# qucontrol/krotov

Hardware: AMD Instinct MI355X
Metric: state*timestep propagations/s (Krotov iterations/s in iterations_per_sec), 256-objective N=64 ensemble (higher is better)
Workload: dtype f64

## Files before the change

krotov_amd/csrc/kh_instances.inc:

```
#if KH_TU == KH_TU_MAIN
extern template __global__ void kh_coop_sweep_store<16, 16, false>(KhSweepArgs, KhCoopArgs, KhExchange, double const*, HIP_vector_type<double, 2u> const*, HIP_vector_type<double, 2u>*, HIP_vector_type<double, 2u>*, int);
extern template __global__ void kh_coop_sweep_store<16, 2, false>(KhSweepArgs, KhCoopArgs, KhExchange, double const*, HIP_vector_type<double, 2u> const*, HIP_vector_type<double, 2u>*, HIP_vector_type<double, 2u>*, int);
extern template __global__ void kh_coop_sweep_store<16, 2, true>(KhSweepArgs, KhCoopArgs, KhExchange, double const*, HIP_vector_type<double, 2u> const*, HIP_vector_type<double, 2u>*, HIP_vector_type<double, 2u>*, int);
extern template __global__ void kh_coop_sweep_store<16, 4, false>(KhSweepArgs, KhCoopArgs, KhExchange, double const*, HIP_vector_type<double, 2u> const*, HIP_vector_type<double, 2u>*, HIP_vector_type<double, 2u>*, int);
extern template __global__ void kh_coop_sweep_store<16, 4, true>(KhSweepArgs, KhCoopArgs, KhExchange, double const*, HIP_vector_type<double, 2u> const*, HIP_vector_type<double, 2u>*, HIP_vector_type<double, 2u>*, int);
extern template __global__ void kh_coop_sweep_store<8, 16, false>(KhSweepArgs, KhCoopArgs, KhExchange, double const*, HIP_vector_type<double, 2u> const*, HIP_vector_type<double, 2u>*, HIP_vector_type<double, 2u>*, int);
extern template __global__ void kh_coop_sweep_store<8, 16, true>(KhSweepArgs, KhCoopArgs, KhExchange, double const*, HIP_vector_type<double, 2u> const*, HIP_vector_type<double, 2u>*, HIP_vector_type<double, 2u>*, int);
extern template __global__ void kh_coop_sweep_store<8, 2, false>(KhSweepArgs, KhCoopArgs, KhExchange, double const*, HIP_vector_type<double, 2u> const*, HIP_vector_type<double, 2u>*, HIP_vector_type<double, 2u>*, int);
extern template __global__ void kh_coop_sweep_store<8, 2, true>(KhSweepArgs, KhCoopArgs, KhExchange, double const*, HIP_vector_type<double, 2u> const*, HIP_vector_type<double, 2u>*, HIP_vector_type<double, 2u>*, int);
extern template __global__ void kh_coop_sweep_store<8, 4, false>(KhSweepArgs, KhCoopArgs, KhExchange, double const*, HIP_vector_type<double, 2u> const*, HIP_vector_type<double, 2u>*, HIP_vector_type<double, 2u>*, int);
extern template __global__ void kh_coop_sweep_store<8, 4, true>(KhSweepArgs, KhCoopArgs, KhExchange, double const*, HIP_vector_type<double, 2u> const*, HIP_vector_type<double, 2u>*, HIP_vector_type<double, 2u>*, int);
extern template __global__ void kh_coop_forward_update<16, 16, false, false, false, true>(KhSweepArgs, KhCoopArgs, KhUpdateArgs, KhExchange);
extern template __global__ void kh_coop_forward_update<16, 2, false, false, false, true>(KhSweepArgs, KhCoopArgs, KhUpdateArgs, KhExchange);
extern template __global__ void kh_coop_forward_update<16, 2, false, true, true, false>(KhSweepArgs, KhCoopArgs, KhUpdateArgs, KhExchange);
extern template __global__ void kh_coop_forward_update<16, 2, true, false, false, true>(KhSweepArgs, KhCoopArgs, KhUpdateArgs, KhExchange);
extern template __global__ void kh_coop_forward_update<16, 4, false, false, false, true>(KhSweepArgs, KhCoopArgs, KhUpdateArgs, KhExchange);
extern template __global__ void kh_coop_forward_update<16, 4, false, true, true, false>(KhSweepArgs, KhCoopArgs, KhUpdateArgs, KhExchange);
extern template __global__ void kh_coop_forward_update<16, 4, true, false, false, true>(KhSweepArgs, KhCoopArgs, KhUpdateArgs, KhExchange);
extern template __global__ void kh_coop_forward_update<8, 16, false, false, false, true>(KhSweepArgs, KhCoopArgs, KhUpdateArgs, KhExchange);
extern template __global__ void kh_coop_forward_update<8, 16, false, true, true, false>(KhSweepArgs, KhCoopArgs, KhUpdateArgs, KhExchange);
extern template __global__ void kh_coop_forward_update<8, 16, true, false, false, true>(KhSweepArgs, KhCoopArgs, KhUpdateArgs, KhExchange);
extern template __global__ void kh_coop_forward_update<8, 2, false, false, false, true>(KhSweepArgs, KhCoopArgs, KhUpdateArgs, KhExchange);
extern template __global__ void kh_coop_forward_update<8, 2, false, true, true, false>(KhSweepArgs, KhCoopArgs, KhUpdateArgs, KhExchange);
extern template __global__ void kh_coop_forward_update<8, 2, true, false, false, true>(KhSweepArgs, KhCoopArgs, KhUpdateArgs, KhExchange);
// ... 75 lines not shown
extern template __global__ void kh_lind_forward_update<2>(KhSweepArgs, KhLindArgs, KhUpdateArgs, KhExchange);
extern template __global__ void kh_lind_forward_update<4>(KhSweepArgs, KhLindArgs, KhUpdateArgs, KhExchange);
extern template __global__ void kh_lind_sweep_store<1>(KhSweepArgs, KhLindArgs, double const*, HIP_vector_type<double, 2u> const*, HIP_vector_type<double, 2u>*, HIP_vector_type<double, 2u>*, int);
extern template __global__ void kh_lind_sweep_store<2>(KhSweepArgs, KhLindArgs, double const*, HIP_vector_type<double, 2u> const*, HIP_vector_type<double, 2u>*, HIP_vector_type<double, 2u>*, int);
extern template __global__ void kh_lind_sweep_store<4>(KhSweepArgs, KhLindArgs, double const*, HIP_vector_type<double, 2u> const*, HIP_vector_type<double, 2u>*, HIP_vector_type<double, 2u>*, int);
extern template __global__ void kh_mini_forward_update<false>(KhSweepArgs, HIP_vector_type<double, 2u> const* const*, KhUpdateArgs, KhExchange);
extern template __global__ void kh_mini_forward_update<true>(KhSweepArgs, HIP_vector_type<double, 2u> const* const*, KhUpdateArgs, KhExchange);
extern template __global__ void kh_quad_forward_update<false>(KhSweepArgs, HIP_vector_type<double, 2u> const* const*, KhUpdateArgs, KhExchange);
extern template __global__ void kh_quad_forward_update<true>(KhSweepArgs, HIP_vector_type<double, 2u> const* const*, KhUpdateArgs, KhExchange);
extern template __global__ void kh_q2_forward_update<false, false, false>(KhSweepArgs, HIP_vector_type<double, 2u> const* const*, KhUpdateArgs, KhExchange);
extern template __global__ void kh_q2_forward_update<false, false, true>(KhSweepArgs, HIP_vector_type<double, 2u> const* const*, KhUpdateArgs, KhExchange);
extern template __global__ void kh_q2_forward_update<false, true, false>(KhSweepArgs, HIP_vector_type<double, 2u> const* const*, KhUpdateArgs, KhExchange);
extern template __global__ void kh_q2_forward_update<false, true, true>(KhSweepArgs, HIP_vector_type<double, 2u> const* const*, KhUpdateArgs, KhExchange);
extern template __global__ void kh_q2_forward_update<true, false, false>(KhSweepArgs, HIP_vector_type<double, 2u> const* const*, KhUpdateArgs, KhExchange);
extern template __global__ void kh_q2_forward_update<true, false, true>(KhSweepArgs, HIP_vector_type<double, 2u> const* const*, KhUpdateArgs, KhExchange);
extern template __global__ void kh_stream_forward_update<1, false, false>(KhSweepArgs, KhUpdateArgs, KhExchange);
extern template __global__ void kh_stream_forward_update<1, false, true>(KhSweepArgs, KhUpdateArgs, KhExchange);
extern template __global__ void kh_stream_forward_update<1, true, false>(KhSweepArgs, KhUpdateArgs, KhExchange);
extern template __global__ void kh_stream_forward_update<1, true, true>(KhSweepArgs, KhUpdateArgs, KhExchange);
extern template __global__ void kh_stream_forward_update<2, false, false>(KhSweepArgs, KhUpdateArgs, KhExchange);
extern template __global__ void kh_stream_forward_update<2, false, true>(KhSweepArgs, KhUpdateArgs, KhExchange);
extern template __global__ void kh_stream_forward_update<2, true, false>(KhSweepArgs, KhUpdateArgs, KhExchange);
extern template __global__ void kh_stream_forward_update<2, true, true>(KhSweepArgs, KhUpdateArgs, KhExchange);
extern template __global__ void kh_stream_forward_update<3, false, false>(KhSweepArgs, KhUpdateArgs, KhExchange);
extern template __global__ void kh_stream_forward_update<3, false, true>(KhSweepArgs, KhUpdateArgs, KhExchange);
extern template __global__ void kh_stream_forward_update<3, true, false>(KhSweepArgs, KhUpdateArgs, KhExchange);
extern template __global__ void kh_stream_forward_update<3, true, true>(KhSweepArgs, KhUpdateArgs, KhExchange);
extern template __global__ void kh_stream_forward_update<4, false, false>(KhSweepArgs, KhUpdateArgs, KhExchange);
extern template __global__ void kh_stream_forward_update<4, false, true>(KhSweepArgs, KhUpdateArgs, KhExchange);
extern template __global__ void kh_stream_forward_update<4, true, false>(KhSweepArgs, KhUpdateArgs, KhExchange);
// ... 162 lines not shown
template __global__ void kh_lind_sweep_store<1>(KhSweepArgs, KhLindArgs, double const*, HIP_vector_type<double, 2u> const*, HIP_vector_type<double, 2u>*, HIP_vector_type<double, 2u>*, int);
template __global__ void kh_lind_sweep_store<2>(KhSweepArgs, KhLindArgs, double const*, HIP_vector_type<double, 2u> const*, HIP_vector_type<double, 2u>*, HIP_vector_type<double, 2u>*, int);
template __global__ void kh_lind_sweep_store<4>(KhSweepArgs, KhLindArgs, double const*, HIP_vector_type<double, 2u> const*, HIP_vector_type<double, 2u>*, HIP_vector_type<double, 2u>*, int);
#elif KH_TU == KH_TU_MINI
template __global__ void kh_mini_forward_update<false>(KhSweepArgs, HIP_vector_type<double, 2u> const* const*, KhUpdateArgs, KhExchange);
template __global__ void kh_mini_forward_update<true>(KhSweepArgs, HIP_vector_type<double, 2u> const* const*, KhUpdateArgs, KhExchange);
template __global__ void kh_quad_forward_update<false>(KhSweepArgs, HIP_vector_type<double, 2u> const* const*, KhUpdateArgs, KhExchange);
template __global__ void kh_quad_forward_update<true>(KhSweepArgs, HIP_vector_type<double, 2u> const* const*, KhUpdateArgs, KhExchange);
#elif KH_TU == KH_TU_Q2
template __global__ void kh_q2_forward_update<false, false, false>(KhSweepArgs, HIP_vector_type<double, 2u> const* const*, KhUpdateArgs, KhExchange);
template __global__ void kh_q2_forward_update<false, false, true>(KhSweepArgs, HIP_vector_type<double, 2u> const* const*, KhUpdateArgs, KhExchange);
template __global__ void kh_q2_forward_update<false, true, false>(KhSweepArgs, HIP_vector_type<double, 2u> const* const*, KhUpdateArgs, KhExchange);
template __global__ void kh_q2_forward_update<false, true, true>(KhSweepArgs, HIP_vector_type<double, 2u> const* const*, KhUpdateArgs, KhExchange);
template __global__ void kh_q2_forward_update<true, false, false>(KhSweepArgs, HIP_vector_type<double, 2u> const* const*, KhUpdateArgs, KhExchange);
template __global__ void kh_q2_forward_update<true, false, true>(KhSweepArgs, HIP_vector_type<double, 2u> const* const*, KhUpdateArgs, KhExchange);
#elif KH_TU == KH_TU_STREAM
template __global__ void kh_stream_forward_update<1, false, false>(KhSweepArgs, KhUpdateArgs, KhExchange);
template __global__ void kh_stream_forward_update<1, false, true>(KhSweepArgs, KhUpdateArgs, KhExchange);
template __global__ void kh_stream_forward_update<1, true, false>(KhSweepArgs, KhUpdateArgs, KhExchange);
template __global__ void kh_stream_forward_update<1, true, true>(KhSweepArgs, KhUpdateArgs, KhExchange);
template __global__ void kh_stream_forward_update<2, false, false>(KhSweepArgs, KhUpdateArgs, KhExchange);
template __global__ void kh_stream_forward_update<2, false, true>(KhSweepArgs, KhUpdateArgs, KhExchange);
template __global__ void kh_stream_forward_update<2, true, false>(KhSweepArgs, KhUpdateArgs, KhExchange);
template __global__ void kh_stream_forward_update<2, true, true>(KhSweepArgs, KhUpdateArgs, KhExchange);
template __global__ void kh_stream_forward_update<3, false, false>(KhSweepArgs, KhUpdateArgs, KhExchange);
template __global__ void kh_stream_forward_update<3, false, true>(KhSweepArgs, KhUpdateArgs, KhExchange);
template __global__ void kh_stream_forward_update<3, true, false>(KhSweepArgs, KhUpdateArgs, KhExchange);
template __global__ void kh_stream_forward_update<3, true, true>(KhSweepArgs, KhUpdateArgs, KhExchange);
template __global__ void kh_stream_forward_update<4, false, false>(KhSweepArgs, KhUpdateArgs, KhExchange);
template __global__ void kh_stream_forward_update<4, false, true>(KhSweepArgs, KhUpdateArgs, KhExchange);
// ... 58 lines not shown
```

krotov_amd/csrc/kh_tile64q2.h:

```cpp
#pragma once

#include "kh_common.h"
#include "kh_generic.h"
#include "kh_tile64.h"

#define KH_Q2_THREADS 512
#ifdef KH_Q2_DPP_REDUCE
typedef KhLanes<false> KhQ2Lanes;
#else
typedef KhLanes<true> KhQ2Lanes;
#endif
#define KH_Q2_TILE_ELEMS (8 * KH_Q2_THREADS)

struct KhQ2Lds {
    cplx *h0;
    cplx *p0;
    cplx (*buf)[KH_TILE_N];
    cplx *chib;
    cplx *sbuf;
    double *red;
    double *D;
    double2 *inv2;
    double *deg;
};

__host__ __device__ inline size_t kh_q2_lds_bytes() {
    return (size_t)2 * KH_Q2_TILE_ELEMS * sizeof(cplx) + 4 * KH_TILE_N * sizeof(cplx) + (2 * 8 * 2 + 4) * sizeof(double) +
           (KH_MAX_DEGREE / 2 + 1) * sizeof(double2) + (KH_MAX_DEGREE + 2) * sizeof(double);
}

__device__ __forceinline__ KhQ2Lds kh_q2_carve(char *smem) {
    KhQ2Lds s;
    s.h0 = (cplx *)smem;
    s.p0 = s.h0 + KH_Q2_TILE_ELEMS;
    s.buf = (cplx(*)[KH_TILE_N])(s.p0 + KH_Q2_TILE_ELEMS);
    s.chib = (cplx *)(s.buf + 2);
    s.sbuf = s.chib + KH_TILE_N;
    s.red = (double *)(s.sbuf + KH_TILE_N);
    s.D = s.red + 2 * 8 * 2;
    s.inv2 = (double2 *)(s.D + 4);
    s.deg = (double *)(s.inv2 + KH_MAX_DEGREE / 2 + 1);
    return s;
}

__device__ __forceinline__ void kh_q2_load_tile(const cplx *op, int N, int wave, int lane, cplx (&t)[8]) {
    const int row = wave * 8 + KhQ2Lanes::row_in(lane), cg = KhQ2Lanes::cg(lane);
#pragma unroll
    for (int j = 0; j < 8; ++j) {
        const int col = cg + 8 * j;
        t[j] = (op != nullptr && row < N && col < N) ? op[(size_t)row * N + col] : c_make(0.0, 0.0);
    }
}

__device__ __forceinline__ void kh_q2_stage_tile(const cplx *op, int N, int wave, int lane, int tid, cplx *dst) {
    cplx t[8];
    kh_q2_load_tile(op, N, wave, lane, t);
// ... 47 lines not shown

__device__ __forceinline__ void kh_q2_advance(const KhQ2Lds &s, int tid, double eps, double eps_prev, const cplx (&h1)[8],
                                              cplx (&a)[8], cplx (&b)[8]) {
    const double e1 = eps - eps_prev, e2 = e1 * (eps + eps_prev);
#pragma unroll
    for (int j = 0; j < 8; ++j) {
        const cplx q1 = s.h0[j * KH_Q2_THREADS + tid];
        const cplx q2 = s.p0[j * KH_Q2_THREADS + tid];
        a[j].x = fma(e1, h1[j].x, a[j].x);
        a[j].y = fma(e1, h1[j].y, a[j].y);
        b[j].x = fma(e2, q2.x, fma(e1, q1.x, b[j].x));
        b[j].y = fma(e2, q2.y, fma(e1, q1.y, b[j].y));
    }
}

template <class Epilogue>
__device__ __forceinline__ int kh_q2_expm_action(const cplx (&a)[8], const cplx (&b)[8], cplx &state,
                                                 cplx (*buf)[KH_TILE_N], cplx *sbuf, const double2 *inv2, int &cur,
                                                 cplx *store_in, int N, double fre, double fim,
                                                 double dt, int nsub, int m, int wave, int lane,
                                                 Epilogue epilogue) {
    const int cg = KhQ2Lanes::cg(lane), row = wave * 8 + KhQ2Lanes::row_out(lane);
    const bool writer = (lane & 7) == 0;
    const double h = nsub == 1 ? dt : dt / nsub;
    const double f2h2 = (fre * fre - fim * fim) * h * h;
    const int phases = (m + 1) >> 1;
    if (store_in != nullptr && wave == 0 && lane < N) {
        store_in[lane] = buf[cur][lane];
    }
    for (int sub = 0; sub < nsub; ++sub) {
        const double hr = h * inv2[0].x, c0 = inv2[KH_Q2_ROWS].x;
        cplx sacc = c_make(hr * state.x, hr * state.y);
        state = c_make(c0 * state.x, c0 * state.y);
        if (phases == 1) {
            if (writer) sbuf[row] = sacc;
            __syncthreads();
        }
        for (int ph = 0; ph < phases; ++ph) {
            const double c2 = f2h2 * inv2[ph].y;
            cplx xv[8];
#pragma unroll
            for (int j = 0; j < 8; ++j) xv[j] = buf[cur][cg + 8 * j];
            const bool last = (ph + 1 == phases);
            cplx yb = c_make(0.0, 0.0);
#pragma unroll
            for (int j = 0; j < 8; ++j) c_fma(yb, b[j], xv[j]);
            const double t2x = KhQ2Lanes::rowsum(yb.x, c2), t2y = KhQ2Lanes::rowsum(yb.y, c2);
            state.x += t2x;
            state.y += t2y;
            if (!last) {
                const double hn = h * inv2[ph + 1].x;
                sacc.x = fma(hn, t2x, sacc.x);
                sacc.y = fma(hn, t2y, sacc.y);
                if (writer) {
                    buf[cur ^ 1][row] = c_make(t2x, t2y);
                    if (ph + 2 == phases) sbuf[row] = sacc;
                }
            } else {
                __builtin_amdgcn_sched_barrier(0);
                cplx sv[8];
#pragma unroll
                for (int j = 0; j < 8; ++j) sv[j] = sbuf[cg + 8 * j];
                cplx ya = c_make(0.0, 0.0);
#pragma unroll
                for (int j = 0; j < 8; ++j) c_fma(ya, a[j], sv[j]);
                const cplx odd = c_mul(c_make(fre, fim), c_make(KhQ2Lanes::rowsum(ya.x, 1.0), KhQ2Lanes::rowsum(ya.y, 1.0)));
                state.x += odd.x;
                state.y += odd.y;
// ... 86 lines not shown
        if (tid == 0 && k == 0 && p.stats != nullptr) {
            p.stats[1] = (double)t_build;
            p.stats[2] = (double)t_phases;
        }
#endif
        if (store != nullptr && wave == 0 && lane < N)
            store[((size_t)k * nt + (direction > 0 ? nt - 1 : 0)) * N + lane] = s.buf[cur][lane];
        if (state_out != nullptr && wave == 0 && lane < N) state_out[(size_t)k * N + lane] = s.buf[cur][lane];
    }
    if (tid == 0 && p.stats != nullptr) atomicAdd(p.stats, matvecs);
}
#else
    ;
#endif

template <bool SO, bool ADJ, bool SINGLE = false>
__global__ void __launch_bounds__(KH_Q2_THREADS)
kh_q2_forward_update(KhSweepArgs p, const cplx *const *__restrict__ sq, KhUpdateArgs u, KhExchange ex) {
    static_assert(!(SO && ADJ), "the second-order bra depends on the new state");
#ifdef KH_Q2_NO_PREFETCH
    constexpr bool PREFETCH = false;
#else
    constexpr bool PREFETCH = !SO;
#endif
    if (u.n_dev != nullptr) {
        u.n_begin = *u.n_dev;
        u.n_end = u.n_begin + 1;
        if (u.n_begin >= p.nt - 1) return;
    }
    extern __shared__ __attribute__((aligned(16))) char smem[];
    const KhQ2Lds s = kh_q2_carve(smem);
    double(*red)[8][2] = (double(*)[8][2])s.red;
    double(*D_sh)[2] = (double(*)[2])s.D;
    const int tid = threadIdx.x, wave = tid >> 6, lane = tid & 63, cg = KhQ2Lanes::cg(lane);
// ... 11 lines not shown
    kh_q2_stage_tile(sq_k[2], N, wave, lane, tid, s.p0);
    cplx h1[8], a[8], b[8];
    kh_q2_load_tile(ops_k[1], N, wave, lane, h1);
    double eps_prev = 0.0;
    const double nrm0 = kh_uniform(p.op_norms[(size_t)k * 2]), nrm1 = kh_uniform(p.op_norms[(size_t)k * 2 + 1]);
    const double chi_norm = kh_uniform(u.chi_norms[k]);

    cplx state = row < N ? u.phi[(size_t)k * N + row] : c_make(0.0, 0.0);
    int cur = 0;
    if (writer) s.buf[0][row] = state;
    __syncthreads();

    double g_a_loc = 0.0;
    cplx chi = c_make(0.0, 0.0), prev = c_make(0.0, 0.0);
    double hs = 0.0;
    auto load_chi = [&](int n) {
        chi = row < N ? u.chi_store[((size_t)k * nt + n) * N + row] : c_make(0.0, 0.0);
        if constexpr (SO) {
            prev = row < N ? u.fw_prev[((size_t)k * nt + n) * N + row] : c_make(0.0, 0.0);
            hs = 0.5 * u.sigma[n] / chi_norm;
        }
    };

    auto partial_pieces = [&](int par) {
        cplx xv[8];
#pragma unroll
        for (int j = 0; j < 8; ++j) xv[j] = s.buf[cur][cg + 8 * j];
        cplx y = c_make(0.0, 0.0);
#pragma unroll
        for (int j = 0; j < 8; ++j) c_fma(y, h1[j], xv[j]);
        y.x = KhQ2Lanes::rowsum(y.x, 1.0);
        y.y = KhQ2Lanes::rowsum(y.y, 1.0);
// ... 31 lines not shown
    }
    if constexpr (ADJ) {
        if (u.n_begin + 1 < nt - 1) {
            load_chi(u.n_begin + 1);
            if (writer) s.chib[row] = chi;
        }
    }
    __syncthreads();

    double dt_next = kh_uniform(p.dt[u.n_begin]), guess_next = kh_uniform(u.guess[u.n_begin]),
           shape_next = kh_uniform(u.shape[u.n_begin]);
    const double lam = kh_uniform(u.lambda[0]);
    int m_rows = -1;
    double stepw_next = kh_uniform(shape_next / lam);
    KhDegreeCache dc = {12, 1.0, 0.0};

#ifdef KH_TIMING
    long long t_ex = 0, t_prop = 0, t_part = 0, t_coll = 0;
    const long long t_all0 = clock64();
#endif
    for (int nr = u.n_begin, n_stop; nr < u.n_end; nr = n_stop) {
    kh_q2_load_tile(ops_k[0], N, wave, lane, a);
    kh_q2_load_tile(sq_k[0], N, wave, lane, b);
    eps_prev = 0.0;
    n_stop = (nr / KH_Q2_REFRESH + 1) * KH_Q2_REFRESH;
    n_stop = n_stop < u.n_end ? n_stop : u.n_end;
    for (int n = nr; n < n_stop; ++n) {
        const int par = n & 1;
        if constexpr (!ADJ) {
            if (n + 1 < nt - 1) load_chi(n + 1);
        }
#ifdef KH_TIMING
        const long long tq0 = clock64();
#endif
        cplx q1[8], q2[8];
        {
            double part[1] = {0.0};
            if (wave == 0) {
                part[0] = partial_total(par);
#ifndef KH_Q2_X_NOEXCH
                kh_exchange_publish(ex, n, k, 1, lane, part);
#endif
            }
            if constexpr (PREFETCH) {
#pragma unroll
                for (int j = 0; j < 8; ++j) {
                    q1[j] = s.h0[j * KH_Q2_THREADS + tid];
                    q2[j] = s.p0[j * KH_Q2_THREADS + tid];
                }
            }
            if constexpr (ADJ) {
                if (n + 1 < nt - 1) adjoint_side();
            }
            if (wave == 0) {
                double D[1];
#ifdef KH_Q2_X_NOEXCH
                const bool ok = true;
                D[0] = part[0];
#else
#ifdef KH_TIMING
                const long long tc0 = clock64();
#endif
                const bool ok = kh_exchange_collect<1, KH_GATHER_CHUNKS, !SINGLE>(ex, n, k, 1, lane, part, D);
#ifdef KH_TIMING
                t_coll += clock64() - tc0;
#endif
#endif
                if (lane == 0) {
                    D_sh[par][0] = D[0];
                    D_sh[par][1] = ok ? 1.0 : 0.0;
                }
            }
        }
        const double dt = dt_next, guess = guess_next, stepw = stepw_next;
        double dt_ld = 0.0, guess_ld = 0.0, shape_ld = 0.0;
        if (n + 1 < nt - 1) {
            dt_ld = p.dt[n + 1];
            guess_ld = u.guess[n + 1];
// ... 10 lines not shown
        g_a_loc = kh_uniform(g_a_loc + stepw * (d1 * d1) * dt);
        dt_next = kh_uniform(dt_ld);
        guess_next = kh_uniform(guess_ld);
        shape_next = kh_uniform(shape_ld);
        if (k == 0 && tid == 0) u.opt[n] = eps;
        int nsub, m;
        kh_degree_cached((nrm0 + fabs(eps) * nrm1) * dt, s.deg, p.theta_max, p.inv_theta_max, dc, &nsub, &m);
        if (m != m_rows) {
            kh_q2_load_rows(p, s, m, tid);
            m_rows = m;
        }
        if constexpr (PREFETCH)
            kh_q2_advance_reg(eps, eps_prev, h1, q1, q2, a, b);
        else
            kh_q2_advance(s, tid, eps, eps_prev, h1, a, b);
        eps_prev = eps;
        stepw_next = kh_uniform(shape_next / lam);
        cplx *fw_out = nullptr;
        if constexpr (SO) fw_out = u.fw_store + ((size_t)k * nt + n) * N;
        if constexpr (ADJ) {
            if (n + 2 < nt - 1) load_chi(n + 2);
            auto epilogue = [&] {
                if (n + 1 < nt - 1) {
                    cplx ov = c_make(0.0, 0.0);
                    if (writer) c_fma_conj(ov, w, state);
                    const double v = KhQ2Lanes::writers_sum(u.mu_re * ov.y + u.mu_im * ov.x);
                    if (lane == 0) red[(n + 1) & 1][wave][0] = v;
                    if (n + 2 < nt - 1 && writer) s.chib[row] = chi;
                }
            };
#ifdef KH_Q2_X_NOPHASES
            epilogue();
            __syncthreads();
#else
            matvecs += kh_q2_expm_action(a, b, state, s.buf, s.sbuf, s.inv2, cur, fw_out, N, p.fre, p.fim, dt, nsub, m, wave,
                                         lane, epilogue);
#endif
        } else {
            matvecs += kh_q2_expm_action(a, b, state, s.buf, s.sbuf, s.inv2, cur, fw_out, N, p.fre, p.fim, dt, nsub, m, wave,
                                         lane, [] {});
        }
#ifdef KH_TIMING
        const long long tq2 = clock64();
        t_prop += tq2 - tq1;
#endif
        if constexpr (!ADJ) {
            if (n + 1 < nt - 1) {
                partial_pieces((n + 1) & 1);
                __syncthreads();
            }
        }
// ... 3 lines not shown
    }
    }
#ifdef KH_TIMING
    if (tid == 0 && k == 0 && p.stats != nullptr) {
        p.stats[1] = (double)t_ex;
        p.stats[2] = (double)t_prop;
        p.stats[3] = (double)t_coll;
    }
#endif
    if (wave == 0 && lane < N) {
        u.phi[(size_t)k * N + lane] = s.buf[cur][lane];
        if constexpr (SO) u.fw_store[((size_t)k * nt + u.n_end) * N + lane] = s.buf[cur][lane];
    }
    if (k == 0 && tid == 0) u.g_a[0] = g_a_loc;
    if (tid == 0 && p.stats != nullptr) atomicAdd(p.stats, matvecs);
}

__global__ void kh_q2_product(const cplx *__restrict__ X, const cplx *__restrict__ Y, cplx *__restrict__ C, int N,
                              int symmetrize)
#if KH_DEFINES(KH_TU_MAIN)
{
    for (int idx = blockIdx.x * blockDim.x + threadIdx.x; idx < N * N; idx += gridDim.x * blockDim.x) {
        const int i = idx / N, j = idx % N;
        cplx acc = c_make(0.0, 0.0);
        for (int q = 0; q < N; ++q) c_fma(acc, X[(size_t)i * N + q], Y[(size_t)q * N + j]);
        if (symmetrize)
            for (int q = 0; q < N; ++q) c_fma(acc, Y[(size_t)i * N + q], X[(size_t)q * N + j]);
        C[idx] = acc;
    }
}
// ... 4 lines not shown
```

krotov_amd/csrc/krotov_hip.hip:

```cpp
#include <hip/hip_runtime.h>

#include <cxxabi.h>
#include <dlfcn.h>

#include <cmath>
#include <cstdarg>
#include <cstdio>
#include <cstdlib>
#include <algorithm>
#include <atomic>
#include <climits>
#include <cstring>
#include <deque>
#include <map>
#include <mutex>
#include <set>
#include <string>
#include <tuple>
#include <type_traits>
#include <utility>
#include <vector>

#include "../../include/krotov_hip.h"
#include "kh_common.h"
// ... 33 lines not shown
        hipError_t _e = (call);                                                               \
        if (_e != hipSuccess)                                                                 \
            return kh_fail(KH_ERR_HIP, "%s failed: %s (%s:%d)", #call, hipGetErrorString(_e), \
                           __FILE__, __LINE__);                                               \
    } while (0)

enum KernelKind { KIND_GENERIC = 0, KIND_TILE_RPT2 = 1, KIND_TILE_RPT1 = 2, KIND_TILE_Q2 = 3, KIND_COOP = 4, KIND_ELL = 5, KIND_TILEN = 6, KIND_TILEX = 7 , KIND_LIND = 8  };

struct KhSwitches {
    std::string kernel;
    bool kernel_set = false;
    bool kernel_is(const char *name) const { return kernel_set && kernel == name; }
    bool taylor, no_adj, near_imag, ellstream, stepwise, stream, coop_xcd, coop_sq, coop_adj, tn_h1reg, tx, q2_store, ens2, gen_adj;
    double ell_cap;
    int stream_G, coop_cols, ens, ens_min_k, ens_ncg;
    bool coop_launch, q2_single, tile_single, coop_single, poll_delay_set, timeout_set;
    int poll_delay, adj_poll_delay, coop_poll_delay;
    long long timeout_ticks;
    int p2p_fail_at, p2p_fail_rank, p2p_fail_sweep;
};

static KhSwitches read_switches() {
    auto on = [](const char *name) { const char *d = getenv(name); return d != nullptr && atoi(d) != 0; };
    auto off = [](const char *name) { const char *d = getenv(name); return d != nullptr && atoi(d) == 0; };
    auto num = [](const char *name, int dflt) { const char *d = getenv(name); return d != nullptr ? atoi(d) : dflt; };
    KhSwitches s;
    if (const char *d = getenv("KH_KERNEL")) s.kernel = d, s.kernel_set = true;
    s.taylor = on("KH_TAYLOR");
    s.no_adj = on("KH_NO_ADJ");
    s.near_imag = !off("KH_NEAR_IMAG");
    s.ell_cap = 0.0;
// ... 4 lines not shown
    s.stream_G = num("KH_STREAM_G", 0);
    s.coop_cols = num("KH_COOP_COLS", 0);
    s.coop_xcd = !off("KH_COOP_XCD");
    s.coop_sq = !on("KH_COOP_NOSQ");
    s.coop_adj = !on("KH_COOP_NO_ADJ");
    s.tn_h1reg = !off("KH_TN_H1REG");
    s.tx = !off("KH_TX");
    s.q2_store = !off("KH_Q2_STORE");
    s.ens = num("KH_ENS", -1);
    s.ens_min_k = num("KH_ENS_MINK", 257);
    s.ens_ncg = num("KH_ENS_NCG", 0);
    s.ens2 = !off("KH_ENS2");
    s.gen_adj = !off("KH_GEN_ADJ");
    s.coop_launch = !off("KH_COOP_LAUNCH");
    s.q2_single = !off("KH_Q2_SINGLE");
    s.tile_single = !off("KH_TILE_SINGLE");
    s.coop_single = !off("KH_COOP_SINGLE");
    s.poll_delay_set = getenv("KH_POLL_DELAY") != nullptr;
    s.poll_delay = num("KH_POLL_DELAY", 16);
    s.adj_poll_delay = num("KH_ADJ_DELAY", 0);
    s.coop_poll_delay = num("KH_COOP_DELAY", 0);
    s.timeout_ticks = 100000000LL;
    s.timeout_set = false;
    if (const char *d = getenv("KH_TIMEOUT_MS"))
        if (atoll(d) > 0) s.timeout_ticks = atoll(d) * 100000LL, s.timeout_set = true;
    s.p2p_fail_at = num("KH_P2P_FAIL_AT", -1);
    s.p2p_fail_rank = num("KH_P2P_FAIL_RANK", 0);
    s.p2p_fail_sweep = num("KH_P2P_FAIL_SWEEP", 1);
    return s;
}

struct KhFacts {
    int K, N, L, num_cus;
    bool csr, shared;
    bool has_h1, all_h1;
    bool ell = false, ell_stream = false;
    int ell_E = 0;
    int ens_ncg = 0;
    double adj_sign = 0.0;
    bool real_spectrum = false;
    double imag_defect = -1.0;
    double theta_max;
    bool lind = false;
};

struct KhPlan {
    KernelKind kind = KIND_GENERIC;
    KernelKind kind_store = KIND_GENERIC;
    int max_wgs = 0, grid_update = 0;
    bool mini = false, quad = false;
    bool stepwise_only = false, stream = false;
    int stream_G = 0;
    int coop_G = 0, coop_Y = 0, coop_ks = 0, coop_cols = KH_COOP_COLS;
    bool coop_xcd = false, coop_sq = false, coop_adj = false, coop_series = false;
    bool tilen = false, tn_h1reg = false;
// ... 63 lines not shown
    cplx *d_phi = nullptr;
    kh_u64 *d_slots = nullptr;
    size_t slots_bytes = 0;
    unsigned int *d_abort = nullptr;
    unsigned long long *d_wait_ticks = nullptr;
    double *d_stats = nullptr;
    double *d_wg_partial = nullptr;
    double *d_step_partial = nullptr;
    cplx *d_gen_scratch = nullptr;
    int gen_scratch_wgs = 0;
    bool gen_scratch_failed = false;
    cplx *d_gen_adj = nullptr;
    bool gen_adj_failed = false;
    bool gen_adj_ready = false;
    double adj_sign = 0.0;
    const double *guess_dev = nullptr;
    const cplx *so_fw_prev = nullptr;
    cplx *so_fw_store = nullptr;
    const double *so_sigma = nullptr;
    int p2p_world = 1, p2p_rank = 0;
    kh_u64 *p2p_window = nullptr;
    size_t p2p_window_bytes = 0;
    std::vector<void *> p2p_opened;
    kh_u64 **d_p2p_peers = nullptr;
    unsigned int p2p_epoch_base = 0;
    bool p2p_ready = false;
    int p2p_sweeps = 0;
    double last_intervals = 0, last_wgs = 0;
    int last_update_grid = 0;
    int reduced_G = 0;
// ... 613 lines not shown
    if (err == hipSuccess) {
        launch(d);
        err = hipGetLastError();
    }
    if (err == hipSuccess) err = hipMemcpy(out, d, bytes, hipMemcpyDeviceToHost);
    (void)hipFree(d);
    KH_HIP(err);
    return KH_OK;
}

template <class Fro2>
static int classify_operators(const kh_engine *e, const kh_problem *pr, bool ctl_plus, bool ctl_minus, bool drift_plus,
                              Fro2 &&fro2, KhFacts &f) {
    f.adj_sign = ctl_plus ? 1.0 : (ctl_minus ? -1.0 : 0.0);
    f.real_spectrum = ctl_plus && drift_plus && !e->is_super;
    if (e->is_super ? ctl_minus : ctl_plus) {
        double v = 0.0, dt_max = 0.0;
        KH_TRY(fro2(v));
        for (int n = 0; n < e->nt - 1; ++n) dt_max = pr->dt[n] > dt_max ? pr->dt[n] : dt_max;
        f.imag_defect = sqrt(v) * dt_max;
    }
    return KH_OK;
}

static int detect_dense(kh_engine *e, const kh_problem *pr, KhFacts &f) {
    const int nops = e->K * (1 + e->L);
    int flags[3] = {1, 1, 1};
    KH_TRY(device_probe(flags, sizeof(flags), [&](void *d) {
        kh_adjoint_sign_kernel<<<(unsigned)(nops < 1024 ? nops : 1024), 256>>>(e->d_ops_fw, e->d_ops_bw, nops, 1 + e->L, e->N, (int *)d);
    }));
// ... 233 lines not shown
    if (e->L >= 1) {
        KH_TRY(csr_fw == nullptr ? detect_dense(e, pr, f) : build_sparse(e, pr, csr_fw, csr_bw, fw, f));
        if (e->sw.taylor) f.real_spectrum = false, f.imag_defect = -1.0;
        if (e->sw.no_adj && csr_fw == nullptr) f.adj_sign = 0.0;
    } else if (csr_fw != nullptr) {
        KH_TRY(build_sparse(e, pr, csr_fw, csr_bw, fw, f));
    }
    if (!e->gen_fits && !f.ell)
        return kh_fail(KH_ERR_UNSUPPORTED, "N=%d: rows wider than 32 entries and no room for the generic kernels' vectors in LDS", e->N);
    if (const int ncg = ens_candidate(f, e->sw)) {
        bool found = false;
        KH_TRY(detect_ensemble(e, fw, found));
        if (found) f.ens_ncg = ncg;
    }
    e->adj_sign = f.adj_sign;

    e->plan = plan_families(f, e->sw);
    KhPlan &p = e->plan;
    if (p.tilen) {
        auto permute = [&](const cplx *src, cplx *dst) {
            kh_tn_permute<<<KH_TN_NMAX / 4, KH_TN_THREADS>>>(src, dst, e->N);
            return KH_OK;
        };
        const size_t bytes = sizeof(cplx) * (KH_TN_NMAX / 4) * KH_TN_THREADS;
        KhCopies copies;
        KH_TRY(stage_copies(e, copies, fw, bytes, nullptr, permute, &e->d_tn_fw));
        KH_TRY(stage_copies(e, copies, bw, bytes, nullptr, permute, &e->d_tn_bw));
    }
    if (p.tx) {
        auto permute = [&](const cplx *src, cplx *dst) {
// ... 3 lines not shown
        const size_t bytes = sizeof(cplx) * 8 * KH_TX_THREADS;
        cplx *zero_tile = nullptr;
        KH_TRY(dev_alloc(e, &zero_tile, bytes));
        KH_HIP(hipMemset(zero_tile, 0, bytes));
        KhCopies copies;
        KH_TRY(stage_copies(e, copies, fw, bytes, zero_tile, permute, &e->d_tx_fw));
        KH_TRY(stage_copies(e, copies, bw, bytes, zero_tile, permute, &e->d_tx_bw));
    }
    std::vector<const cplx *> sq[2];
    if (p.stage_sq) KH_TRY(stage_squares(e, fw, bw, sq));
    if (p.kind == KIND_COOP) KH_TRY(stage_coop(e, fw, bw, sq));
    KH_TRY(stage_series(e));
    if (p.kind_store == KIND_TILE_Q2)
        KH_HIP(hipFuncSetAttribute((const void *)kh_q2_sweep_store, hipFuncAttributeMaxDynamicSharedMemorySize, (int)kh_q2_lds_bytes()));
    if (p.kind == KIND_TILE_Q2) {
        const void *forms[] = {(const void *)kh_q2_forward_update<false, true, true>, (const void *)kh_q2_forward_update<false, false, true>,
                               (const void *)kh_q2_forward_update<true, false, true>, (const void *)kh_q2_forward_update<false, true>,
                               (const void *)kh_q2_forward_update<false, false>,      (const void *)kh_q2_forward_update<true, false>};
        for (const void *fn : forms)
            KH_HIP(hipFuncSetAttribute(fn, hipFuncAttributeMaxDynamicSharedMemorySize, (int)kh_q2_lds_bytes()));
        int rc = KH_OK;
        if (!p.mini && e->K > 1)
            for (const void *fn : forms)
                if (rc == KH_OK) rc = check_residency(e, fn, KH_Q2_THREADS, kh_q2_lds_bytes(), e->K, "kh_q2_forward_update");
        if (rc != KH_OK) {
            p.kind = KIND_GENERIC;
            p.grid_update = e->K < p.max_wgs ? e->K : p.max_wgs;
        }
    }
    if (p.ens) {
        e->ens_H0 = fw[0];
// ... 678 lines not shown
            launch_plain<kh_mini_forward_update<SO>>(dim3(1), dim3(64 * e->K), 0, st, p, e->d_sq_fw, u, ex);
        return KH_OK;
    });
}

static int update_q2(kh_engine *e, const KhSweepArgs &p, const KhUpdateArgs &u, const KhExchange &ex, hipStream_t st) {
    const dim3 g(e->K), b(KH_Q2_THREADS);
    const size_t lds = kh_q2_lds_bytes();
    const bool single = ex.world == 1 && e->sw.q2_single;
    if (u.sigma != nullptr)
        return single ? launch_persistent<kh_q2_forward_update<true, false, true>>(e, g, b, lds, st, p, e->d_sq_fw, u, ex)
                      : launch_persistent<kh_q2_forward_update<true, false>>(e, g, b, lds, st, p, e->d_sq_fw, u, ex);
    if (u.adj_sign != 0.0) {
        KhExchange exa = ex;
        exa.first_poll_delay = e->sw.adj_poll_delay;
        return single ? launch_persistent<kh_q2_forward_update<false, true, true>>(e, g, b, lds, st, p, e->d_sq_fw, u, exa)
                      : launch_persistent<kh_q2_forward_update<false, true>>(e, g, b, lds, st, p, e->d_sq_fw, u, exa);
    }
    return single ? launch_persistent<kh_q2_forward_update<false, false, true>>(e, g, b, lds, st, p, e->d_sq_fw, u, ex)
                  : launch_persistent<kh_q2_forward_update<false, false>>(e, g, b, lds, st, p, e->d_sq_fw, u, ex);
}

static int update_tilen(kh_engine *e, const KhSweepArgs &p, const KhUpdateArgs &u, const KhExchange &ex, hipStream_t st) {
    const bool so = u.sigma != nullptr;
    KhUpdateArgs ut = u;
    if (!so && !e->plan.tn_h1reg && ensure_gen_adj(e)) {
        KH_TRY(gen_adjoint_side(e, u.chi_store, e->L, st));
        ut.adj_store = e->d_gen_adj;
    }
    KhExchange ext = ex;
// ... 613 lines not shown
```

Baseline: 65.71 million.

## Publish adjoint overlap early inside the q2 expm series for Hermitian single-GPU runs

Adds an early-publish variant of the q2 forward update kernel. It computes the next step's control overlap <chi|mu|psi> incrementally as Taylor terms of the propagator are produced. It precomputes the auxiliary products A·chi and H1·chi into LDS so that the exchange partial can be published before the series finishes, shortening the cross-block collect wait on the critical path. It costs extra matvecs, more LDS per block, and added register pressure, and it is gated on Hermitian, single-GPU and nsub==1 conditions.

```diff
diff --git a/krotov_amd/csrc/kh_instances.inc b/krotov_amd/csrc/kh_instances.inc
--- a/krotov_amd/csrc/kh_instances.inc
+++ b/krotov_amd/csrc/kh_instances.inc
@@ -113,6 +113,7 @@
 extern template __global__ void kh_q2_forward_update<false, true, true>(KhSweepArgs, HIP_vector_type<double, 2u> const* const*, KhUpdateArgs, KhExchange);
 extern template __global__ void kh_q2_forward_update<true, false, false>(KhSweepArgs, HIP_vector_type<double, 2u> const* const*, KhUpdateArgs, KhExchange);
 extern template __global__ void kh_q2_forward_update<true, false, true>(KhSweepArgs, HIP_vector_type<double, 2u> const* const*, KhUpdateArgs, KhExchange);
+extern template __global__ void kh_q2_forward_update_early<true>(KhSweepArgs, HIP_vector_type<double, 2u> const* const*, KhUpdateArgs, KhExchange);
 extern template __global__ void kh_stream_forward_update<1, false, false>(KhSweepArgs, KhUpdateArgs, KhExchange);
 extern template __global__ void kh_stream_forward_update<1, false, true>(KhSweepArgs, KhUpdateArgs, KhExchange);
 extern template __global__ void kh_stream_forward_update<1, true, false>(KhSweepArgs, KhUpdateArgs, KhExchange);
@@ -305,6 +306,7 @@
 template __global__ void kh_q2_forward_update<false, true, true>(KhSweepArgs, HIP_vector_type<double, 2u> const* const*, KhUpdateArgs, KhExchange);
 template __global__ void kh_q2_forward_update<true, false, false>(KhSweepArgs, HIP_vector_type<double, 2u> const* const*, KhUpdateArgs, KhExchange);
 template __global__ void kh_q2_forward_update<true, false, true>(KhSweepArgs, HIP_vector_type<double, 2u> const* const*, KhUpdateArgs, KhExchange);
+template __global__ void kh_q2_forward_update_early<true>(KhSweepArgs, HIP_vector_type<double, 2u> const* const*, KhUpdateArgs, KhExchange);
 #elif KH_TU == KH_TU_STREAM
 template __global__ void kh_stream_forward_update<1, false, false>(KhSweepArgs, KhUpdateArgs, KhExchange);
 template __global__ void kh_stream_forward_update<1, false, true>(KhSweepArgs, KhUpdateArgs, KhExchange);
diff --git a/krotov_amd/csrc/kh_tile64q2.h b/krotov_amd/csrc/kh_tile64q2.h
--- a/krotov_amd/csrc/kh_tile64q2.h
+++ b/krotov_amd/csrc/kh_tile64q2.h
@@ -22,11 +22,13 @@
     double *D;
     double2 *inv2;
     double *deg;
+    cplx *wbuf;
+    cplx (*ubuf)[KH_TILE_N];
 };
 
 __host__ __device__ inline size_t kh_q2_lds_bytes() {
     return (size_t)2 * KH_Q2_TILE_ELEMS * sizeof(cplx) + 4 * KH_TILE_N * sizeof(cplx) + (2 * 8 * 2 + 4) * sizeof(double) +
-           (KH_MAX_DEGREE / 2 + 1) * sizeof(double2) + (KH_MAX_DEGREE + 2) * sizeof(double);
+           (KH_MAX_DEGREE / 2 + 1) * sizeof(double2) + (KH_MAX_DEGREE + 2) * sizeof(double) + 3 * KH_TILE_N * sizeof(cplx);
 }
 
 __device__ __forceinline__ KhQ2Lds kh_q2_carve(char *smem) {
@@ -40,6 +42,8 @@
     s.D = s.red + 2 * 8 * 2;
     s.inv2 = (double2 *)(s.D + 4);
     s.deg = (double *)(s.inv2 + KH_MAX_DEGREE / 2 + 1);
+    s.wbuf = (cplx *)(s.deg + KH_MAX_DEGREE + 2);
+    s.ubuf = (cplx(*)[KH_TILE_N])(s.wbuf + KH_TILE_N);
     return s;
 }
 
@@ -117,12 +121,35 @@
     }
 }
 
-template <class Epilogue>
+struct KhQ2NoEarly {
+    static constexpr bool on = false;
+};
+template <class Reduce, class Publish>
+struct KhQ2EarlySum {
+    static constexpr bool on = true;
+    bool active;
+    const cplx *wvec;
+    cplx w, fwp;
+    Reduce reduce;
+    Publish publish;
+    cplx y = {0.0, 0.0}, acc = {0.0, 0.0};
+    __device__ __forceinline__ void term(double g, double hc, double tx, double ty) {
+        const cplx coef = c_make(fma(hc, fwp.x, g * w.x), fma(hc, fwp.y, g * w.y));
+        c_fma_conj(acc, coef, c_make(tx, ty));
+    }
+};
+template <class Reduce, class Publish>
+__device__ __forceinline__ KhQ2EarlySum<Reduce, Publish> kh_q2_early_sum(bool active, const cplx *wvec, cplx w, cplx fwp,
+                                                                         Reduce reduce, Publish publish) {
+    return KhQ2EarlySum<Reduce, Publish>{active, wvec, w, fwp, reduce, publish};
+}
+
+template <class Epilogue, class Early = KhQ2NoEarly>
 __device__ __forceinline__ int kh_q2_expm_action(const cplx (&a)[8], const cplx (&b)[8], cplx &state,
                                                  cplx (*buf)[KH_TILE_N], cplx *sbuf, const double2 *inv2, int &cur,
                                                  cplx *store_in, int N, double fre, double fim,
                                                  double dt, int nsub, int m, int wave, int lane,
-                                                 Epilogue epilogue) {
+                                                 Epilogue epilogue, Early early = Early()) {
     const int cg = KhQ2Lanes::cg(lane), row = wave * 8 + KhQ2Lanes::row_out(lane);
     const bool writer = (lane & 7) == 0;
     const double h = nsub == 1 ? dt : dt / nsub;
@@ -134,6 +161,9 @@
     for (int sub = 0; sub < nsub; ++sub) {
         const double hr = h * inv2[0].x, c0 = inv2[KH_Q2_ROWS].x;
         cplx sacc = c_make(hr * state.x, hr * state.y);
+        if constexpr (Early::on) {
+            if (early.active) early.term(c0, hr, state.x, state.y);
+        }
         state = c_make(c0 * state.x, c0 * state.y);
         if (phases == 1) {
             if (writer) sbuf[row] = sacc;
@@ -145,16 +175,42 @@
 #pragma unroll
             for (int j = 0; j < 8; ++j) xv[j] = buf[cur][cg + 8 * j];
             const bool last = (ph + 1 == phases);
+            if constexpr (Early::on) {
+                if (early.active && last) early.publish();
+            }
             cplx yb = c_make(0.0, 0.0);
 #pragma unroll
             for (int j = 0; j < 8; ++j) c_fma(yb, b[j], xv[j]);
             const double t2x = KhQ2Lanes::rowsum(yb.x, c2), t2y = KhQ2Lanes::rowsum(yb.y, c2);
             state.x += t2x;
             state.y += t2y;
+            if constexpr (Early::on) {
+                if (early.active && ph == 0) {
+                    __builtin_amdgcn_sched_barrier(0);
+                    const cplx *wvec = early.wvec + kh_launder(cg);
+                    cplx wv[8];
+#pragma unroll
+                    for (int j = 0; j < 8; ++j) wv[j] = wvec[8 * j];
+                    cplx yw = c_make(0.0, 0.0);
+#pragma unroll
+                    for (int j = 0; j < 8; ++j) c_fma(yw, b[j], wv[j]);
+                    early.y = c_make(KhQ2Lanes::rowsum(yw.x, 1.0), KhQ2Lanes::rowsum(yw.y, 1.0));
+                }
+            }
             if (!last) {
                 const double hn = h * inv2[ph + 1].x;
                 sacc.x = fma(hn, t2x, sacc.x);
                 sacc.y = fma(hn, t2y, sacc.y);
+                if constexpr (Early::on) {
+                    if (early.active) {
+                        early.term(1.0, hn, t2x, t2y);
+                        if (ph + 2 == phases) {
+                            const double c2n = f2h2 * inv2[ph + 1].y;
+                            c_fma_conj(early.acc, c_make(c2n * early.y.x, c2n * early.y.y), c_make(t2x, t2y));
+                            early.reduce(early.acc);
+                        }
+                    }
+                }
                 if (writer) {
                     buf[cur ^ 1][row] = c_make(t2x, t2y);
                     if (ph + 2 == phases) sbuf[row] = sacc;
@@ -271,10 +327,11 @@
     ;
 #endif
 
-template <bool SO, bool ADJ, bool SINGLE = false>
-__global__ void __launch_bounds__(KH_Q2_THREADS)
-kh_q2_forward_update(KhSweepArgs p, const cplx *const *__restrict__ sq, KhUpdateArgs u, KhExchange ex) {
+template <bool SO, bool ADJ, bool SINGLE, bool EARLY>
+__device__ __forceinline__ void kh_q2_update_body(KhSweepArgs p, const cplx *const *__restrict__ sq, KhUpdateArgs u,
+                                                  KhExchange ex) {
     static_assert(!(SO && ADJ), "the second-order bra depends on the new state");
+    static_assert(!EARLY || (ADJ && SINGLE), "the early sum is the adjoint-side sum; built for one GPU only");
 #ifdef KH_Q2_NO_PREFETCH
     constexpr bool PREFETCH = false;
 #else
@@ -316,8 +373,12 @@
     double g_a_loc = 0.0;
     cplx chi = c_make(0.0, 0.0), prev = c_make(0.0, 0.0);
     double hs = 0.0;
+    auto in_place = [](int v) {
+        if constexpr (EARLY) return kh_launder(v);
+        return v;
+    };
     auto load_chi = [&](int n) {
-        chi = row < N ? u.chi_store[((size_t)k * nt + n) * N + row] : c_make(0.0, 0.0);
+        chi = row < N ? u.chi_store[((size_t)k * nt + n) * N + in_place(row)] : c_make(0.0, 0.0);
         if constexpr (SO) {
             prev = row < N ? u.fw_prev[((size_t)k * nt + n) * N + row] : c_make(0.0, 0.0);
             hs = 0.5 * u.sigma[n] / chi_norm;
@@ -379,6 +440,7 @@
     int m_rows = -1;
     double stepw_next = kh_uniform(shape_next / lam);
     KhDegreeCache dc = {12, 1.0, 0.0};
+    [[maybe_unused]] bool published = false;
 
 #ifdef KH_TIMING
     long long t_ex = 0, t_prop = 0, t_part = 0, t_coll = 0;
@@ -404,10 +466,17 @@
             if (wave == 0) {
                 part[0] = partial_total(par);
 #ifndef KH_Q2_X_NOEXCH
-                kh_exchange_publish(ex, n, k, 1, lane, part);
-#endif
-            }
-            if constexpr (PREFETCH) {
+                if constexpr (EARLY) {
+                    if (!published) kh_exchange_publish(ex, n, k, 1, lane, part);
+                } else {
+                    kh_exchange_publish(ex, n, k, 1, lane, part);
+                }
+#endif
+            }
+            if constexpr (PREFETCH && EARLY) {
+#pragma unroll
+                for (int j = 0; j < 8; ++j) q1[j] = s.h0[j * KH_Q2_THREADS + tid];
+            } else if constexpr (PREFETCH) {
 #pragma unroll
                 for (int j = 0; j < 8; ++j) {
                     q1[j] = s.h0[j * KH_Q2_THREADS + tid];
@@ -416,6 +485,35 @@
             }
             if constexpr (ADJ) {
                 if (n + 1 < nt - 1) adjoint_side();
+            }
+            if constexpr (EARLY) {
+                if (writer) s.wbuf[kh_launder(row)] = w;
+                __syncthreads();
+                if (n + 1 < nt - 1) {
+                    const cplx *wvec = s.wbuf + kh_launder(cg);
+                    cplx xv[8];
+#pragma unroll
+                    for (int j = 0; j < 8; ++j) xv[j] = wvec[8 * j];
+                    cplx y1 = c_make(0.0, 0.0), y2 = c_make(0.0, 0.0);
+#pragma unroll
+                    for (int j = 0; j < 8; ++j) {
+                        c_fma(y1, a[j], xv[j]);
+                        c_fma(y2, h1[j], xv[j]);
+                    }
+                    y1 = c_make(KhQ2Lanes::rowsum(y1.x, 1.0), KhQ2Lanes::rowsum(y1.y, 1.0));
+                    y2 = c_make(KhQ2Lanes::rowsum(y2.x, 1.0), KhQ2Lanes::rowsum(y2.y, 1.0));
+                    if (writer) {
+                        cplx *urow = s.ubuf[0] + kh_launder(row);
+                        urow[0] = y1;
+                        urow[KH_TILE_N] = y2;
+                    }
+                    matvecs += 2.0;
+                }
+                if constexpr (PREFETCH) {
+                    __builtin_amdgcn_sched_barrier(0);
+#pragma unroll
+                    for (int j = 0; j < 8; ++j) q2[j] = s.p0[j * KH_Q2_THREADS + tid];
+                }
             }
             if (wave == 0) {
                 double D[1];
@@ -426,7 +524,7 @@
 #ifdef KH_TIMING
                 const long long tc0 = clock64();
 #endif
-                const bool ok = kh_exchange_collect<1, KH_GATHER_CHUNKS, !SINGLE>(ex, n, k, 1, lane, part, D);
+                const bool ok = kh_exchange_collect<1, KH_GATHER_CHUNKS, !SINGLE>(ex, n, k, 1, in_place(lane), part, D);
 #ifdef KH_TIMING
                 t_coll += clock64() - tc0;
 #endif
@@ -467,18 +565,30 @@
             kh_q2_advance_reg(eps, eps_prev, h1, q1, q2, a, b);
         else
             kh_q2_advance(s, tid, eps, eps_prev, h1, a, b);
+        cplx fwp = c_make(0.0, 0.0);
+        if constexpr (EARLY) {
+            const double de = eps - eps_prev;
+            const cplx *urow = s.ubuf[0] + kh_launder(row);
+            const cplx u1 = urow[0], u2 = urow[KH_TILE_N];
+            w = s.wbuf[kh_launder(row)];
+            const cplx wp = c_make(fma(de, u2.x, u1.x), fma(de, u2.y, u1.y));
+            fwp = c_make(p.fre * wp.x + p.fim * wp.y, p.fre * wp.y - p.fim * wp.x);
+        }
         eps_prev = eps;
         stepw_next = kh_uniform(shape_next / lam);
         cplx *fw_out = nullptr;
         if constexpr (SO) fw_out = u.fw_store + ((size_t)k * nt + n) * N;
         if constexpr (ADJ) {
             if (n + 2 < nt - 1) load_chi(n + 2);
+            const bool early_now = EARLY && nsub == 1 && m >= 3 && n + 1 < u.n_end;
             auto epilogue = [&] {
                 if (n + 1 < nt - 1) {
-                    cplx ov = c_make(0.0, 0.0);
-                    if (writer) c_fma_conj(ov, w, state);
-                    const double v = KhQ2Lanes::writers_sum(u.mu_re * ov.y + u.mu_im * ov.x);
-                    if (lane == 0) red[(n + 1) & 1][wave][0] = v;
+                    if (!early_now) {
+                        cplx ov = c_make(0.0, 0.0);
+                        if (writer) c_fma_conj(ov, w, state);
+                        const double v = KhQ2Lanes::writers_sum(u.mu_re * ov.y + u.mu_im * ov.x);
+                        if (lane == 0) red[(n + 1) & 1][wave][0] = v;
+                    }
                     if (n + 2 < nt - 1 && writer) s.chib[row] = chi;
                 }
             };
@@ -486,8 +596,25 @@
             epilogue();
             __syncthreads();
 #else
-            matvecs += kh_q2_expm_action(a, b, state, s.buf, s.sbuf, s.inv2, cur, fw_out, N, p.fre, p.fim, dt, nsub, m, wave,
-                                         lane, epilogue);
+            if constexpr (EARLY) {
+                auto reduce = [&](const cplx &ov) {
+                    const double v = KhQ2Lanes::writers_sum(writer ? u.mu_re * ov.y + u.mu_im * ov.x : 0.0);
+                    if (lane == 0) red[(n + 1) & 1][wave][0] = v;
+                };
+                auto publish = [&] {
+                    if (wave == 0) {
+                        double part[1] = {partial_total((n + 1) & 1)};
+                        kh_exchange_publish(ex, n + 1, k, 1, lane, part);
+                    }
+                };
+                matvecs += kh_q2_expm_action(a, b, state, s.buf, s.sbuf, s.inv2, cur, fw_out, N, p.fre, p.fim, dt, nsub, m,
+                                             wave, lane, epilogue, kh_q2_early_sum(early_now, s.wbuf, w, fwp, reduce, publish));
+                if (early_now) matvecs += 1.0;
+                published = early_now;
+            } else {
+                matvecs += kh_q2_expm_action(a, b, state, s.buf, s.sbuf, s.inv2, cur, fw_out, N, p.fre, p.fim, dt, nsub, m,
+                                             wave, lane, epilogue);
+            }
 #endif
         } else {
             matvecs += kh_q2_expm_action(a, b, state, s.buf, s.sbuf, s.inv2, cur, fw_out, N, p.fre, p.fim, dt, nsub, m, wave,
@@ -521,6 +648,17 @@
     }
     if (k == 0 && tid == 0) u.g_a[0] = g_a_loc;
     if (tid == 0 && p.stats != nullptr) atomicAdd(p.stats, matvecs);
+}
+
+template <bool SO, bool ADJ, bool SINGLE = false>
+__global__ void __launch_bounds__(KH_Q2_THREADS)
+kh_q2_forward_update(KhSweepArgs p, const cplx *const *__restrict__ sq, KhUpdateArgs u, KhExchange ex) {
+    kh_q2_update_body<SO, ADJ, SINGLE, false>(p, sq, u, ex);
+}
+template <bool SINGLE>
+__global__ void __launch_bounds__(KH_Q2_THREADS)
+kh_q2_forward_update_early(KhSweepArgs p, const cplx *const *__restrict__ sq, KhUpdateArgs u, KhExchange ex) {
+    kh_q2_update_body<false, true, SINGLE, true>(p, sq, u, ex);
 }
 
 __global__ void kh_q2_product(const cplx *__restrict__ X, const cplx *__restrict__ Y, cplx *__restrict__ C, int N,
diff --git a/krotov_amd/csrc/krotov_hip.hip b/krotov_amd/csrc/krotov_hip.hip
--- a/krotov_amd/csrc/krotov_hip.hip
+++ b/krotov_amd/csrc/krotov_hip.hip
@@ -71,7 +71,7 @@
     bool taylor, no_adj, near_imag, ellstream, stepwise, stream, coop_xcd, coop_sq, coop_adj, tn_h1reg, tx, q2_store, ens2, gen_adj;
     double ell_cap;
     int stream_G, coop_cols, ens, ens_min_k, ens_ncg;
-    bool coop_launch, q2_single, tile_single, coop_single, poll_delay_set, timeout_set;
+    bool coop_launch, q2_single, q2_early, tile_single, coop_single, poll_delay_set, timeout_set;
     int poll_delay, adj_poll_delay, coop_poll_delay;
     long long timeout_ticks;
     int p2p_fail_at, p2p_fail_rank, p2p_fail_sweep;
@@ -106,6 +106,7 @@
     s.gen_adj = !off("KH_GEN_ADJ");
     s.coop_launch = !off("KH_COOP_LAUNCH");
     s.q2_single = !off("KH_Q2_SINGLE");
+    s.q2_early = !off("KH_Q2_EARLY");
     s.tile_single = !off("KH_TILE_SINGLE");
     s.coop_single = !off("KH_COOP_SINGLE");
     s.poll_delay_set = getenv("KH_POLL_DELAY") != nullptr;
@@ -131,6 +132,7 @@
     int ens_ncg = 0;
     double adj_sign = 0.0;
     bool real_spectrum = false;
+    bool hermitian = false;
     double imag_defect = -1.0;
     double theta_max;
     bool lind = false;
@@ -224,6 +226,7 @@
     bool gen_adj_failed = false;
     bool gen_adj_ready = false;
     double adj_sign = 0.0;
+    bool hermitian = false;
     const double *guess_dev = nullptr;
     const cplx *so_fw_prev = nullptr;
     cplx *so_fw_store = nullptr;
@@ -867,6 +870,7 @@
                               Fro2 &&fro2, KhFacts &f) {
     f.adj_sign = ctl_plus ? 1.0 : (ctl_minus ? -1.0 : 0.0);
     f.real_spectrum = ctl_plus && drift_plus && !e->is_super;
+    f.hermitian = f.real_spectrum;
     if (e->is_super ? ctl_minus : ctl_plus) {
         double v = 0.0, dt_max = 0.0;
         KH_TRY(fro2(v));
@@ -1130,6 +1134,7 @@
         if (found) f.ens_ncg = ncg;
     }
     e->adj_sign = f.adj_sign;
+    e->hermitian = f.hermitian;
 
     e->plan = plan_families(f, e->sw);
     KhPlan &p = e->plan;
@@ -1163,7 +1168,8 @@
     if (p.kind_store == KIND_TILE_Q2)
         KH_HIP(hipFuncSetAttribute((const void *)kh_q2_sweep_store, hipFuncAttributeMaxDynamicSharedMemorySize, (int)kh_q2_lds_bytes()));
     if (p.kind == KIND_TILE_Q2) {
-        const void *forms[] = {(const void *)kh_q2_forward_update<false, true, true>, (const void *)kh_q2_forward_update<false, false, true>,
+        const void *forms[] = {(const void *)kh_q2_forward_update_early<true>,
+                               (const void *)kh_q2_forward_update<false, true, true>, (const void *)kh_q2_forward_update<false, false, true>,
                                (const void *)kh_q2_forward_update<true, false, true>, (const void *)kh_q2_forward_update<false, true>,
                                (const void *)kh_q2_forward_update<false, false>,      (const void *)kh_q2_forward_update<true, false>};
         for (const void *fn : forms)
@@ -1872,6 +1878,8 @@
     if (u.adj_sign != 0.0) {
         KhExchange exa = ex;
         exa.first_poll_delay = e->sw.adj_poll_delay;
+        if (single && e->hermitian && e->sw.q2_early)
+            return launch_persistent<kh_q2_forward_update_early<true>>(e, g, b, lds, st, p, e->d_sq_fw, u, exa);
         return single ? launch_persistent<kh_q2_forward_update<false, true, true>>(e, g, b, lds, st, p, e->d_sq_fw, u, exa)
                       : launch_persistent<kh_q2_forward_update<false, true>>(e, g, b, lds, st, p, e->d_sq_fw, u, exa);
     }
```

New measurement: 56.75 million. 0.864x the previous value.
